# garrelt/C2-Ray3Dm

Hardware: AMD Instinct MI355X
Metric: cells-traced/sec (grid^3 x sources / wallclock) on 256^3 (higher is better)
Workload: dtype f64

## Files before the change

c2-ray3dm_amd/_capi.py:

```python
import ctypes as C
import os

_HERE = os.path.dirname(os.path.abspath(__file__))
LIB_PATH = os.path.join(_HERE, "libc2ray_hip.so")
MAX_ITER_LOG = 128

GRID_NDENS, GRID_XH, GRID_XH_AV, GRID_XH_INTERMED, GRID_PHIH, GRID_PHIHEAT, GRID_TEMPER, GRID_XH0, GRID_XH_AV0, GRID_XH_INTERMED0 = range(10)


class Params(C.Structure):
    _fields_ = [("mesh", C.c_int32 * 3), ("device", C.c_int32), ("subboxsize", C.c_int32),
                ("max_subbox", C.c_int32), ("numtau", C.c_int32), ("max_outer_iter", C.c_int32),
                ("max_chem_iter", C.c_int32), ("deterministic_rates", C.c_int32),
                ("sweep_mode", C.c_int32), ("allfrac", C.c_int32),
                ("epsilon", C.c_double), ("convergence_fraction", C.c_double),
                ("minimum_fractional_change", C.c_double), ("minimum_fraction_of_atoms", C.c_double),
                ("loss_fraction", C.c_double), ("max_coldensh", C.c_double),
                ("tau_photo_limit", C.c_double), ("sigma_HI", C.c_double),
                ("minlogtau", C.c_double), ("dlogtau", C.c_double), ("weight_floor", C.c_double),
                ("sqrt2", C.c_double), ("sqrt3", C.c_double), ("pi", C.c_double),
                ("abu_c", C.c_double), ("bh00", C.c_double), ("albpow", C.c_double),
                ("colh0", C.c_double), ("temph0", C.c_double), ("S_star", C.c_double),
                ("scratch_bytes", C.c_size_t)]

# ... 55 lines not shown
    ("c2r_set_clumping_grid", C.c_int, [_P, _P]),
    ("c2r_default_thermal", C.c_int, [C.POINTER(ThermalParams)]),
    ("c2r_set_thermal", C.c_int, [_P, C.POINTER(ThermalParams), _P, _P, _I32, _P]),
    ("c2r_set_redshift", C.c_int, [_P, _D]),
    ("c2r_set_final_temperature", C.c_int, [_P]),
    ("c2r_set_sources", C.c_int, [_P, _P, _P, _I32]),
    ("c2r_set_exchange_overlap", C.c_int, [_P, _I32]),
    ("c2r_set_xray_tables", C.c_int, [_P, _P, _P, _I32]),
    ("c2r_set_xray_heat_tables", C.c_int, [_P, _P, _P, _I32]),
    ("c2r_set_xray_sources", C.c_int, [_P, _P, _I32]),
    ("c2r_set_rank", C.c_int, [_P, _I32, _I32, ALLREDUCE_FN, _P]),
    ("c2r_set_slab_chemistry", C.c_int, [_P, _P, _P, _P]),
    ("c2r_slab", C.c_int, [_P, _I32, _I32, C.POINTER(C.c_size_t), C.POINTER(C.c_size_t)]),
    ("c2r_set_source_share", C.c_int, [_P, _P, _I32]),
    ("c2r_last_nbox", C.c_int, [_P, _P, _I32]),
    ("c2r_set_balance", C.c_int, [_P, _I32]),
    ("c2r_source_share", C.c_int, [_P, _P, _I32, C.POINTER(_I32)]),
    ("c2r_balanced_shares", C.c_int, [_P, _I32, _I32, _I32, _P, C.POINTER(_I32)]),
    ("c2r_set_source_queue", C.c_int, [_P, _P, _P, _I32]),
    ("c2r_get_device", C.c_int, [_P, C.POINTER(_I32)]),
    ("c2r_bind_device_buffers", C.c_int, [_P, _P, _P, _P, _P, _P]),
    ("c2r_device_ptr", C.c_int, [_P, _I32, C.POINTER(_P)]),
    ("c2r_upload", C.c_int, [_P, _I32, _P]),
    ("c2r_download", C.c_int, [_P, _I32, _P]),
    ("c2r_zero_rates", C.c_int, [_P]),
    ("c2r_pass_sources", C.c_int, [_P, C.POINTER(_D), C.POINTER(_I64), C.POINTER(_I64)]),
    ("c2r_allreduce_rates", C.c_int, [_P]),
    ("c2r_exchange_stats", C.c_int, [_P, C.POINTER(_I64), C.POINTER(_I64), C.POINTER(_I64), C.POINTER(_I64)]),
    ("c2r_evolve0d_host", C.c_int, [_P, _I32, C.c_void_p, C.c_void_p, C.c_void_p, C.c_void_p, C.c_void_p, C.c_void_p, C.c_void_p,
                                    C.c_void_p, C.POINTER(_D)]),
# ... 96 lines not shown
```

c2-ray3dm_amd/csrc/ctx.hpp:

```cpp
#pragma once
#include "../../include/c2ray_hip.h"
#include "../../include/c2ray_constants.h"
#include "kernels_common.hpp"

#include <algorithm>
#include <chrono>
#include <cmath>
#include <cstdio>
#include <cstring>
#include <functional>
#include <map>
#include <string>
#include <vector>

namespace c2r {

struct BoxDesc;

constexpr int kSumBlocks = 1024;
constexpr int kFoldLossMax = 64;
constexpr int kFusedQmax = 10;
constexpr int kMaxSlabRanks = 64;
constexpr int kFewSources = 32;

constexpr int kMaxChains = 4;
struct SweepScratch {
    hipStream_t stream = nullptr; bool own_stream = false;
    int cap = 0;
    double *d_planes = nullptr;
    double *d_gbox = nullptr;
    double *d_gbox_h = nullptr;
    int *d_srcpos_b = nullptr, *d_srcw_b = nullptr; double *d_nflux_b = nullptr, *d_nflux_x = nullptr;
    char *d_batch = nullptr, *h_batch = nullptr; size_t batch_bytes = 0;
    char *d_batch_init = nullptr; std::vector<char> batch_image;
    char *d_hbatch = nullptr;
    int *d_active[2] = {nullptr, nullptr};
    int *d_nactive = nullptr;
    int *h_nactive = nullptr;
    int *d_hnactive = nullptr;
    std::vector<hipEvent_t> ev_box;
    hipEvent_t ev_done = nullptr;
    double *d_loss_partial = nullptr, *d_loss_acc = nullptr, *d_final_loss = nullptr;
    int *d_final_nbox = nullptr;
    int *d_perm = nullptr, *h_perm = nullptr;
};

struct Ctx {
    c2r_params prm{};
    hipStream_t stream = nullptr;
    bool own_stream = false;
    size_t ncell = 0;
    void *grid[10] = {nullptr, nullptr, nullptr, nullptr, nullptr, nullptr, nullptr, nullptr, nullptr, nullptr};
// ... 8 lines not shown
    bool  own[5] = {false, false, false, false, false};
    double *d_thick = nullptr, *d_thin = nullptr;
    v2f64 *d_logtab = nullptr;
    v2f64 *d_odtab = nullptr;
    bool fast = false;
    bool have_tables = false, have_step = false;
    double dr[3] = {0, 0, 0}, vol = 0, lls = 0, temper = 0;
    float clumping = 1.0f;
    std::vector<int32_t> srcpos;
    std::vector<double>  nflux;
    bool xray = false; std::vector<double> nflux_x; double *d_xthick = nullptr, *d_xthin = nullptr;
    bool have_xheat = false; double *d_xhthick = nullptr, *d_xhthin = nullptr;
    int nsrc = 0, rank = 0, nranks = 1;
    bool explicit_share = false; std::vector<int32_t> share;
    std::vector<int32_t> last_nbox;
    int box_hint = 0;
    struct BatchGraph { hipGraph_t graph = nullptr; hipGraphExec_t exec = nullptr; unsigned long long gen = 0; int count = 0, n_active = 0, hint = 0;
                        bool fused = false; bool stats = false; const void *acc = nullptr;
    };
    std::map<int, BatchGraph> graphs;
    struct ChainGraph { hipGraph_t graph = nullptr; hipGraphExec_t exec = nullptr; unsigned long long gen = 0; int count = 0, n_active = 0, shape_count = 0;
                        const void *acc = nullptr; bool perm = false; int H = 0, launches = 0; std::vector<int> bounds, profile, profile_prev; int passes_since_capture = 0; };
    std::map<int, ChainGraph> chain_graphs;
    bool chain_tail = true;
    bool chain_graph = true;
    long long chain_replays = 0, chain_halts = 0, chain_eager = 0;
    unsigned long long gen = 1;
    long long captures = 0;
    bool use_graph = true;
    bool fused_iter = true;
// ... 125 lines not shown
```

c2-ray3dm_amd/csrc/kernels_sweep.hpp:

```cpp
#pragma once
#include "kernels_common.hpp"

namespace c2r {

template <int EXT>
__device__ __forceinline__ void source_cell(const KParams &p, const v2f64 *__restrict__ ltab, const int s, const bool on_surface,
                                            double *loss_acc, double *dbg_cdout)
{
    const int i = pmod(p.srcpos[3 * s + 0] - 1, p.n[0]);
    const int j = pmod(p.srcpos[3 * s + 1] - 1, p.n[1]);
    const int k = pmod(p.srcpos[3 * s + 2] - 1, p.n[2]);
    const size_t id = (size_t)i + (size_t)p.n[0] * ((size_t)j + (size_t)p.n[1] * (size_t)k);
    const double nhi = p.nhi[id];
    const double cd_in = 0.0;
    const double path = 0.5 * step_of(p).dr[0];
    const double vol_ph = step_of(p).dr[0] * step_of(p).dr[1] * step_of(p).dr[2];
    const double cd_out = cd_in + nhi * path;
    for (int f = 0; f < 6; ++f)
        p.planes[((size_t)s * 2 + 0) * 6 * p.PP + (size_t)f * p.PP + (size_t)p.R * p.P + p.R] = cd_out;
    if (dbg_cdout) dbg_cdout[id] = cd_out;
    const double nflux = p.normflux[s];
    double p_out = 0.0, gamma = 0.0;
    if (nflux > 0.0) {
        double heat = 0.0;
// ... 601 lines not shown
    __shared__ v2f64 s_log[kBlock];
    const int face = blockIdx.y;
    const int tile = blockIdx.x;
    const int nact = *sa.n_active;
    if ((int)blockIdx.z >= nact) return;
    const FaceRect fr = sa.face[face];
    if (tile >= fr.ntiles && !sa.has_boundary) return;
    const v2f64 *ltab = wave_log_table(p.odtab, s_log);
    sweep_tile_fast<DET, LLS, STREAM, EXT>(p, sa, fr, ltab, p.thick, sm, face, tile, (int)blockIdx.z, sa);
}

struct XcdArgs {
    const int *perm;
    int n, cap;
    const int *final_nbox;
};
template <bool DET, int LLS, bool STREAM, int EXT, bool FAST>
__global__ C2R_FAST_ATTR void k_sweep_shell_xcd(KParams p, ShellArgs sa, XcdArgs xa)
{
    __shared__ double sm[16];
    __shared__ v2f64 s_log[kBlock];
    const unsigned x = blockIdx.x & 7u;
    unsigned r = blockIdx.x >> 3;
    const unsigned start = (x * (unsigned)xa.n) >> 3, cnt = (((x + 1u) * (unsigned)xa.n) >> 3) - start;
    int face = -1; unsigned item = 0, tile = 0;
#pragma unroll
    for (int f = 0; f < 6; ++f) {
        const unsigned nt = (unsigned)sa.face[f].ntiles, nb = cnt * nt;
        if (face < 0) {
            if (r < nb) { face = f; item = r / nt; tile = r - item * nt; }
            else r -= nb;
        }
    }
    if (face < 0) return;
    const int s = xa.perm[(2 - (face >> 1)) * xa.cap + (int)(start + item)];
    if (xa.final_nbox[s] != 0) return;
    const FaceRect fr = sa.face[face];
    const v2f64 *ltab = wave_log_table(p.odtab, s_log);
    if (FAST) sweep_tile_fast<DET, LLS, STREAM ? 3 : 2, EXT>(p, sa, fr, ltab, p.thick, sm, face, (int)tile, 0, sa, s);
    else sweep_tile<DET, LLS, STREAM ? 3 : 2, EXT>(p, sa, fr, ltab, sm, face, (int)tile, 0, sa, s);
}

template <bool DET, int LLS, bool STREAM, int EXT>
__global__ __launch_bounds__(kBlock) __attribute__((amdgpu_waves_per_eu(1, 4)))
void k_sweep_pair_fast(KParams p, ShellArgs sa, ShellArgs sb)
{
    __shared__ double sm[16];
    __shared__ v2f64 s_log[kBlock];
    const bool second = blockIdx.y >= 6;
    const int face = second ? (int)blockIdx.y - 6 : (int)blockIdx.y;
    const int tile = blockIdx.x;
    const int nact = *sa.n_active;
    if ((int)blockIdx.z >= nact) return;
    const v2f64 *ltab = (C2R_PAIR_LDS_TABLE) ? wave_log_table(p.odtab, s_log) : p.odtab;
    if (second) {
// ... 214 lines not shown
                                                     int bps, double *loss_acc)
{
    __shared__ double sm[4];
    const int sl = blockIdx.x;
    if (sl >= *n_active) return;
    double v = 0.0;
    for (int i = threadIdx.x; i < bps; i += 256) v += loss_partial[(size_t)sl * bps + i];
    const double tot = block_sum_256(v, sm);
    if (threadIdx.x == 0) loss_acc[active[sl]] += tot;
}

__global__ __launch_bounds__(1024) void k_box_decide(const int *active_in, const int *n_in_dev, int *active_out,
                                                     int *n_out, int *n_out_host, const double *normflux, double S_star,
                                                     double loss_fraction, int can_grow, int nbox,
                                                     double *loss_acc, double *final_loss, int *final_nbox,
                                                     const double *loss_partial, int bps, int next_bound, int *halt_host)
{
    __shared__ int scan[1024];
    __shared__ int base;
    const int n_in = *n_in_dev;
    if (threadIdx.x == 0) base = 0;
    __syncthreads();
    for (int start = 0; start < n_in; start += 1024) {
        const int i = start + (int)threadIdx.x;
        int keep = 0, s = -1;
        if (i < n_in) {
            s = active_in[i];
            const double flux = normflux[s] * S_star;
            double loss = loss_acc[s];
            if (bps > 0) {
                const double *pp = loss_partial + (size_t)i * bps;
// ... 5 lines not shown
                loss_acc[s] = loss;
            }
            keep = (loss > loss_fraction * flux) && can_grow;
            if (keep) loss_acc[s] = 0.0;
            else { final_loss[s] = loss; final_nbox[s] = nbox; }
        }
        scan[threadIdx.x] = keep;
        __syncthreads();
        for (int off = 1; off < 1024; off <<= 1) {
            int v = 0;
            if ((int)threadIdx.x >= off) v = scan[threadIdx.x - off];
            __syncthreads();
            scan[threadIdx.x] += v;
            __syncthreads();
        }
        if (keep) active_out[base + scan[threadIdx.x] - 1] = s;
        __syncthreads();
        if (threadIdx.x == 1023) base += scan[1023];
        __syncthreads();
    }
    if (threadIdx.x == 0) {
        const bool over = base > next_bound;
        *n_out = over ? 0 : base; *n_out_host = base;
        if (over) *halt_host = nbox;
    }
}

struct SmallTotals {
    int on, nsrc;
    double *photon_loss; long long *sum_nbox;
    double *host_loss; long long *host_nbox;
    int *host_final_nbox; double *host_final_loss;
};
__global__ __launch_bounds__(64) void k_box_decide_small(const int *active_in, const int *n_in_dev, int *active_out,
                                                         int *n_out, int *n_out_host, const double *normflux, double S_star,
                                                         double loss_fraction, int can_grow, int nbox,
                                                         double *loss_acc, double *final_loss, int *final_nbox,
                                                         const double *loss_partial, int bps, SmallTotals tot,
                                                         int next_bound, int *halt_host)
{
#if defined(__AMDGCN_WAVEFRONT_SIZE) && __AMDGCN_WAVEFRONT_SIZE != 64
#error "k_box_decide_small is one 64-lane wave (ballot, cross-lane reads of final_loss): build for a wave64 target (gfx950)"
#endif
    const int n_in = *n_in_dev;
    const int i = threadIdx.x;
    int keep = 0, s = -1;
    if (i < n_in) {
        s = active_in[i];
        const double flux = normflux[s] * S_star;
        double loss = loss_acc[s];
        if (bps > 0) {
            const double *pp = loss_partial + (size_t)i * bps;
            double a0 = 0.0, a1 = 0.0, a2 = 0.0, a3 = 0.0;
            int j = 0;
            for (; j + 3 < bps; j += 4) { a0 += pp[j]; a1 += pp[j + 1]; a2 += pp[j + 2]; a3 += pp[j + 3]; }
            for (; j < bps; ++j) a0 += pp[j];
            loss = loss + ((a0 + a1) + (a2 + a3));
            loss_acc[s] = loss;
        }
        keep = (loss > loss_fraction * flux) && can_grow;
        if (keep) loss_acc[s] = 0.0;
        else { final_loss[s] = loss; final_nbox[s] = nbox; }
    }
    const unsigned long long mask = __ballot(keep);
    if (keep) active_out[__popcll(mask & ((1ULL << i) - 1ULL))] = s;
    const int n_keep = __popcll(mask);
    if (i == 0) {
        const bool over = n_keep > next_bound;
        *n_out = over ? 0 : n_keep; *n_out_host = n_keep;
        if (over) *halt_host = nbox;
    }
    if (tot.on && n_keep == 0) {
        __threadfence_block();
        __syncthreads();
        for (int t = i; t < tot.nsrc; t += 64) { tot.host_final_nbox[t] = final_nbox[t]; tot.host_final_loss[t] = final_loss[t]; }
        if (i == 0) {
            double L = 0.0; long long NB = 0;
            for (int t = 0; t < tot.nsrc; ++t) { L = L + (0.0 + final_loss[t]); NB += final_nbox[t]; }
            *tot.photon_loss = L; *tot.sum_nbox = NB;
            *tot.host_loss = L; *tot.host_nbox = NB;
// ... 38 lines not shown
```

c2-ray3dm_amd/csrc/sweep.hip:

```cpp
#include "ctx.hpp"
#include "kernels_sweep.hpp"
#include <climits>

namespace c2r {

namespace {
void free_chain(SweepScratch &sc)
{
    hipFree(sc.d_planes); hipFree(sc.d_gbox); hipFree(sc.d_gbox_h); hipFree(sc.d_batch); hipFree(sc.d_batch_init); hipFree(sc.d_loss_partial);
    hipFree(sc.d_perm);
    if (sc.h_perm) hipHostFree(sc.h_perm);
    if (sc.h_batch) hipHostFree(sc.h_batch);
    if (sc.h_nactive) hipHostFree(sc.h_nactive);
    for (auto &e : sc.ev_box) hipEventDestroy(e);
    if (sc.ev_done) hipEventDestroy(sc.ev_done);
    const hipStream_t st = sc.stream; const bool own = sc.own_stream;
    sc = SweepScratch();
    sc.stream = st; sc.own_stream = own;
}
}

void free_sweep_scratch(Ctx *ctx)
{
    for (int c = 0; c < kMaxChains; ++c) free_chain(ctx->sc[c]);
// ... 11 lines not shown
{
    if (ctx->chains_env > 0) return std::min(ctx->chains_env, std::max(1, want));
    if (ctx->prm.deterministic_rates || want < 64 || want > 768) return 1;
    if (ctx->stream_hint && ctx->xcd_order != 0 &&
        (double)want >= ctx->xcd_min_per_plane * (double)std::min(ctx->prm.mesh[0], std::min(ctx->prm.mesh[1], ctx->prm.mesh[2]))) return 1;
    return (want >= 192 && want <= 384) ? 3 : 2;
}

int alloc_chain(Ctx *ctx, SweepScratch &sc, int cap)
{
    if (!sc.stream) { HIP_TRY(hipStreamCreateWithFlags(&sc.stream, hipStreamNonBlocking)); sc.own_stream = true; }
    HIP_TRY(hipMalloc(&sc.d_planes, (size_t)cap * 2 * 6 * ctx->PP * sizeof(double)));
    if (ctx->prm.deterministic_rates) HIP_TRY(hipMalloc(&sc.d_gbox, (size_t)cap * 2 * ctx->ncell * sizeof(double)));
    if (ctx->prm.deterministic_rates && ctx->thermal) HIP_TRY(hipMalloc(&sc.d_gbox_h, (size_t)cap * 2 * ctx->ncell * sizeof(double)));
    HIP_TRY(hipMalloc(&sc.d_loss_partial, (size_t)cap * 6 * ctx->tiles_cap * sizeof(double)));
    sc.batch_bytes = (size_t)cap * 4 * sizeof(double) + ((size_t)cap * 9 + 2) * sizeof(int);
    HIP_TRY(hipMalloc(&sc.d_batch, sc.batch_bytes));
    HIP_TRY(hipMalloc(&sc.d_batch_init, sc.batch_bytes));
    sc.batch_image.clear();
    HIP_TRY(hipHostMalloc((void **)&sc.h_batch, sc.batch_bytes, hipHostMallocMapped));
    HIP_TRY(hipHostGetDevicePointer((void **)&sc.d_hbatch, sc.h_batch, 0));
    {
        double *d = reinterpret_cast<double *>(sc.d_batch);
        sc.d_nflux_b = d; sc.d_final_loss = d + cap; sc.d_loss_acc = d + 2 * (size_t)cap; sc.d_nflux_x = d + 3 * (size_t)cap;
        int *i = reinterpret_cast<int *>(d + 4 * (size_t)cap);
        sc.d_srcpos_b = i; sc.d_srcw_b = i + 3 * (size_t)cap; sc.d_active[0] = i + 6 * (size_t)cap;
        sc.d_active[1] = i + 7 * (size_t)cap; sc.d_final_nbox = i + 8 * (size_t)cap; sc.d_nactive = i + 9 * (size_t)cap;
    }
    HIP_TRY(hipMalloc(&sc.d_perm, (size_t)3 * cap * sizeof(int)));
    HIP_TRY(hipHostMalloc((void **)&sc.h_perm, (size_t)3 * cap * sizeof(int)));
    HIP_TRY(hipHostMalloc((void **)&sc.h_nactive, (size_t)(ctx->nbox_max + 2) * sizeof(int), hipHostMallocMapped));
    HIP_TRY(hipHostGetDevicePointer((void **)&sc.d_hnactive, sc.h_nactive, 0));
    sc.ev_box.resize(ctx->nbox_max + 2);
    for (auto &e : sc.ev_box) HIP_TRY(hipEventCreateWithFlags(&e, hipEventDisableTiming));
    HIP_TRY(hipEventCreateWithFlags(&sc.ev_done, hipEventDisableTiming));
    sc.cap = cap;
    return C2R_OK;
}
}

int ensure_sweep_scratch(Ctx *ctx, int want)
{
// ... 187 lines not shown
        if ((spins & 63u) == 63u && std::chrono::steady_clock::now() - t0 > std::chrono::microseconds(500)) {
            (void)hipGetLastError();
            HIP_TRY(hipEventSynchronize(ev));
            return C2R_OK;
        }
        cpu_relax();
    }
    (void)hipGetLastError();
    return C2R_OK;
}

struct BatchSweep {
    Ctx *ctx; SweepScratch &sc; const c2r_params &p;
    const int first, count; const bool first_of_pass; double *const dbg; FusedIter *const fz;
    const size_t cap; hipStream_t st; KParams k;
    double *h_nf, *h_fl, *h_nfx; int *h_pos, *h_posw, *h_act, *h_na, *h_fnb;
    int n_active = 0;
    int cur = 0, last_bps = 0;
    int totals_at_box = 0;

    const int shape_count;
    bool chained = false;
    int launches = 0;
    int bound = 0, known = 0;
    int next = 1, last = 0;
    bool perm_ready = false;

    BatchSweep(Ctx *c, SweepScratch &sc_, int first_, int count_, bool first_of_pass_, double *dbg_, FusedIter *fz_)
        : ctx(c), sc(sc_), p(c->prm), first(first_), count(count_), first_of_pass(first_of_pass_), dbg(dbg_), fz(fz_),
          cap((size_t)sc_.cap), st(sc_.stream), k(make_kparams(c, sc_)), shape_count(c->queue_next ? c->nsrc : n_local_sources(c))
    {
        h_nf = reinterpret_cast<double *>(sc.h_batch); h_fl = h_nf + cap; h_nfx = h_nf + 3 * cap;
        h_pos = reinterpret_cast<int *>(h_nf + 4 * cap); h_posw = h_pos + 3 * cap; h_act = h_pos + 6 * cap; h_na = h_pos + 9 * cap;
        h_fnb = h_pos + 8 * cap;
    }

    void stage()
    {
        memset(sc.h_batch, 0, sc.batch_bytes);
        const bool can_trace = ctx->hr[2] > 0 && ctx->hl[2] > 0;
        n_active = 0;
        for (int i = 0; i < count; ++i) {
            const int g = ctx->explicit_share ? ctx->share[first + i]
                                              : ctx->rank + (first + i) * ctx->nranks;
            for (int d = 0; d < 3; ++d) {
                h_pos[3 * i + d] = ctx->srcpos[3 * (size_t)g + d];
                const int m = (h_pos[3 * i + d] - 1) % p.mesh[d];
                h_posw[3 * i + d] = m < 0 ? m + p.mesh[d] : m;
            }
            h_nf[i] = ctx->nflux[g];
            h_nfx[i] = (ctx->xray && g < (int)ctx->nflux_x.size()) ? ctx->nflux_x[g] : 0.0;
            const double flux = h_nf[i] * p.S_star;
            if (flux > p.loss_fraction * flux && can_trace) h_act[n_active++] = i;
            else h_fl[i] = flux;
        }
        h_na[0] = n_active; h_na[1] = 0;
    }

    void stage_perm()
    {
        perm_ready = false;
        if (dbg || !sc.d_perm || ctx->xcd_order == 0 || n_active < ctx->xcd_min_sources) return;
        const int nmin = std::min(p.mesh[0], std::min(p.mesh[1], p.mesh[2]));
        if (ctx->xcd_order < 0 && (double)n_active < ctx->xcd_min_per_plane * (double)nmin * (sc.d_gbox ? 0.5 : 1.0)) return;
        for (int d = 0; d < 3; ++d) {
            int *perm = sc.h_perm + (size_t)d * cap;
            for (int t = 0; t < n_active; ++t) perm[t] = h_act[t];
            std::stable_sort(perm, perm + n_active, [&](int a, int b) { return h_posw[3 * a + d] < h_posw[3 * b + d]; });
// ... 143 lines not shown
                        case 4: C2R_LAUNCH_PAIR(false, 2); break;
                        case 5: C2R_LAUNCH_PAIR(true, 2); break;
                        case 6: C2R_LAUNCH_PAIR(false, 3); break;
                        default: C2R_LAUNCH_PAIR(true, 3); break;
                    }
#undef C2R_LAUNCH_PAIR
#undef C2R_LAUNCH_PAIR_H
                    pbuf = 1 - pbuf;
                    ++q;
                    continue;
                }
            }
            pbuf = 1 - pbuf;
            ++in_box;
            if (prof == 1) prof_begin(ctx, ctx->ev_sweep, ctx->ev_sweep_used);
            if (perm_ready && !sa.has_boundary && q >= ctx->xcd_qmin && (double)bound >= ctx->xcd_min_alive * (double)n_active) {
                XcdArgs xa{};
                xa.perm = sc.d_perm; xa.n = n_active; xa.cap = (int)cap; xa.final_nbox = sc.d_final_nbox;
                int tiles6 = 0;
                for (int f = 0; f < 6; ++f) tiles6 += sa.face[f].ntiles;
                const dim3 grid(8u * (unsigned)((n_active + 7) / 8) * (unsigned)tiles6), blk(kBlock);
#define C2R_LAUNCH_XCD_D(D, L, H, F) do { if (ctx->stream_hint) hipLaunchKernelGGL((k_sweep_shell_xcd<D, L, true, H, F>), grid, blk, 0, st, k, sa, xa); \
                                          else hipLaunchKernelGGL((k_sweep_shell_xcd<D, L, false, H, F>), grid, blk, 0, st, k, sa, xa); } while (0)
#define C2R_LAUNCH_XCD_F(L, H, F) do { if (det) C2R_LAUNCH_XCD_D(true, L, H, F); else C2R_LAUNCH_XCD_D(false, L, H, F); } while (0)
#define C2R_LAUNCH_XCD_H(L, H) do { if (ctx->fast) C2R_LAUNCH_XCD_F(L, H, true); else C2R_LAUNCH_XCD_F(L, H, false); } while (0)
#define C2R_LAUNCH_XCD(L) do { if (ctx->thermal && ctx->xray) C2R_LAUNCH_XCD_H(L, 3); else if (ctx->thermal) C2R_LAUNCH_XCD_H(L, 1); else if (ctx->xray) C2R_LAUNCH_XCD_H(L, 2); else C2R_LAUNCH_XCD_H(L, 0); } while (0)
                switch (ctx->lls_type) {
                    case 1: C2R_LAUNCH_XCD(1); break;
                    case 2: C2R_LAUNCH_XCD(2); break;
                    default: C2R_LAUNCH_XCD(3); break;
                }
#undef C2R_LAUNCH_XCD
#undef C2R_LAUNCH_XCD_H
// ... 35 lines not shown
    {
        const int nbox = bx.nbox;
        int *const halt = sc.d_hnactive;
        const int can_grow = (p.subboxsize * nbox < ctx->hr[2]) && (p.subboxsize * nbox < ctx->hl[2]);
        if (n_active <= 64) {
            SmallTotals tot{};
            if (nbox == totals_at_box) {
                tot.on = 1; tot.nsrc = count; tot.photon_loss = ctx->d_photon_loss; tot.sum_nbox = ctx->d_sum_nbox;
                tot.host_loss = &ctx->d_hsc->photon_loss; tot.host_nbox = &ctx->d_hsc->sum_nbox;
                tot.host_final_loss = reinterpret_cast<double *>(sc.d_hbatch) + cap;
                tot.host_final_nbox = reinterpret_cast<int *>(reinterpret_cast<double *>(sc.d_hbatch) + 4 * cap) + 8 * cap;
            }
            hipLaunchKernelGGL(k_box_decide_small, dim3(1), dim3(64), 0, st, sc.d_active[cur], sc.d_nactive + cur,
                               sc.d_active[1 - cur], sc.d_nactive + (1 - cur), sc.d_hnactive + nbox, sc.d_nflux_b,
                               p.S_star, p.loss_fraction, can_grow, nbox, sc.d_loss_acc, sc.d_final_loss, sc.d_final_nbox,
                               (const double *)sc.d_loss_partial, last_bps, tot, bx.next_bound, halt);
        } else
        hipLaunchKernelGGL(k_box_decide, dim3(1), dim3(1024), 0, st, sc.d_active[cur], sc.d_nactive + cur,
                           sc.d_active[1 - cur], sc.d_nactive + (1 - cur), sc.d_hnactive + nbox, sc.d_nflux_b,
                           p.S_star, p.loss_fraction, can_grow, nbox, sc.d_loss_acc, sc.d_final_loss, sc.d_final_nbox,
                           (const double *)sc.d_loss_partial, last_bps, bx.next_bound, halt);
    }

    int enqueue_box(const int nbox, const int bound, const int next_bound = INT_MAX)
    {
        Box bx{};
        bx.nbox = nbox; bx.bound = bound; bx.next_bound = next_bound;
        for (int d = 0; d < 3; ++d) {
            bx.boxR[d] = std::min(p.subboxsize * nbox, ctx->hr[d]);
            bx.boxL[d] = std::min(p.subboxsize * nbox, ctx->hl[d]);
        }
        bx.pair_ok = ctx->pair_shells && n_active <= kFewSources && !dbg && ctx->prof != 1;
        bx.pbuf = plane_set_before(ctx, nbox, n_active, bx.pair_ok);
        bx.fused_box = box_is_fused(ctx, nbox, bx.pair_ok);
        bx.q0 = p.subboxsize * (nbox - 1) + 1; bx.q1 = std::min(p.subboxsize * nbox, ctx->Qmax);
        bx.det = sc.d_gbox != nullptr;
// ... 164 lines not shown
        cg.perm = perm_ready;
        cg.passes_since_capture = 0;
        return true;
    }
    if (cg.graph) { hipGraphDestroy(cg.graph); cg.graph = nullptr; }
    cg.exec = nullptr;
    (void)hipGetLastError();
    ctx->use_graph = false;
    return false;
}

int sweep_batch(Ctx *ctx, int first, int count, bool first_of_pass, double *dbg, std::vector<int> *nbox_out,
                std::vector<double> *loss_out, FusedIter *fz = nullptr)
{
    BatchSweep bs(ctx, ctx->sc[0], first, count, first_of_pass, dbg, fz);
    return bs.run(nbox_out, loss_out);
}

#ifndef C2R_CHAIN_AHEAD
#define C2R_CHAIN_AHEAD 2
#endif
constexpr int kChainAhead = C2R_CHAIN_AHEAD;

static void bounds_from_profile(const std::vector<int> &prof, int n_active, std::vector<int> &bounds, int &H)
{
    H = 0;
    while (H + 1 < (int)prof.size() && prof[H] > 0) ++H;
    bounds.assign((size_t)H + 1, 0);
    for (int nb = 1; nb <= H; ++nb) {
        const int c = prof[nb - 1];
// ... 14 lines not shown
        have += cg.bounds[nb]; need += cg.profile[nb - 1];
    }
    return have <= need + need / 2 + 4LL * H;
}

static_assert(kFusedQmaxK == kFusedQmax, "the fused kernel's LDS planes are sized for kFusedQmax");
static_assert(kGateChains >= kMaxChains, "k_chain_gate holds every chain's pointers");
int run_chains(Ctx *ctx, int first, int count, bool first_of_pass, std::vector<int> *nbox_out, FusedIter *tail)
{
    const int nch = std::min(ctx->nchains, count);
    const int per = (count + nch - 1) / nch;
    std::vector<BatchSweep> ch;
    ch.reserve(nch);
    for (int c = 0, f = first; c < nch && f < first + count; ++c, f += per)
        ch.emplace_back(ctx, ctx->sc[c], f, std::min(per, first + count - f), first_of_pass && c == 0, nullptr, nullptr);
    HIP_TRY(hipEventRecord(ctx->ev_prepared, ctx->stream));
    if (ctx->prof) prof_begin(ctx, ctx->ev_sweep, ctx->ev_sweep_used);
    std::vector<Ctx::ChainGraph *> graph_of(ch.size(), nullptr);
    for (size_t c = 0; c < ch.size(); ++c) {
        BatchSweep &b = ch[c];
        b.chained = true;
        b.stage();
        if (ctx->xcd_order > 0) b.stage_perm();
        if (b.st != ctx->stream) HIP_TRY(hipStreamWaitEvent(b.st, ctx->ev_prepared, 0));
        b.bound = b.n_active; b.known = 0; b.cur = 0; b.next = 1;
        Ctx::ChainGraph &cg = ctx->chain_graphs[b.first];
        ++cg.passes_since_capture;
        bool replay = false;
        if (ctx->use_graph && ctx->chain_graph && b.n_active > 0 && !cg.profile.empty()) {
            replay = chain_graph_fits(ctx, cg, b, (const void *)b.k.phih);
// ... 207 lines not shown
    ctx->xchg_bytes_total += ctx->xchg_bytes_last;
    return C2R_OK;
}
}

int pass_sources_impl(Ctx *ctx, FusedIter *fz, double *photon_loss, int64_t *sum_nbox, int64_t *visited, bool no_wait, FusedIter *chain_tail)
{
    int rc;
    if ((rc = sync_step(ctx))) return rc;
    const bool queued = ctx->queue_next != nullptr && fz == nullptr;
    if (queued) { ctx->share.clear(); ctx->explicit_share = true; ctx->auto_share = true; }
    else balance_before_pass(ctx);
    int nloc = queued ? 0 : n_local_sources(ctx);
    long long vis = 0;
    ++ctx->pass_id; ctx->sparse_valid = ctx->rates_clean || fz != nullptr; ctx->rates_clean = false;
    ctx->last_nbox.clear();
    ctx->h_sc->photon_loss = 0.0; ctx->h_sc->sum_nbox = 0;
    const bool overlap = !queued && exchange_overlap_applies(ctx, fz);
    if (queued) {
        bool prepared = false;
        std::vector<int> nb;
        for (;;) {
            int32_t qf = 0, qc = 0;
            if (ctx->queue_next(ctx->queue_user, (int64_t)ctx->pass_id, ctx->queue_chunk, &qf, &qc) != 0) FAIL(C2R_ECALLBACK, "source queue callback failed");
            if (qc <= 0) break;
            if (qf < 0 || qc > ctx->queue_chunk || qf + qc > ctx->nsrc) FAIL(C2R_ECALLBACK, "source queue handed out sources beyond the list");
            const int first = (int)ctx->share.size();
            for (int i = 0; i < qc; ++i) ctx->share.push_back(qf + i);
            if ((rc = ensure_sweep_scratch(ctx, ctx->queue_chunk))) return rc;
            if (!prepared) { if ((rc = sweep_prepare(ctx))) return rc; prepared = true; }
            for (int f = first, count = 0; f < first + qc; f += count) {
// ... 60 lines not shown
}

using namespace c2r;

extern "C" {

int c2r_pass_sources(c2r_ctx *c, double *photon_loss, int64_t *sum_nbox, int64_t *visited)
{
    if (!c) return C2R_EINVAL;
    Ctx *ctx = C(c);
    int rc = check_ready(ctx);
    if (rc) return rc;
    return pass_sources_impl(ctx, nullptr, photon_loss, sum_nbox, visited);
}

int c2r_do_source(c2r_ctx *c, int32_t ns, double *cd_host, double *loss, int32_t *nbox, int64_t *visited)
{
    if (!c) return C2R_EINVAL;
    Ctx *ctx = C(c);
    int rc = check_ready(ctx);
    if (rc) return rc;
    if (ns < 1 || ns > ctx->nsrc) FAIL(C2R_EINVAL, "source number out of range");
    rc = ensure_sweep_scratch(ctx, 1);
    if (rc) return rc;
    if ((rc = sync_step(ctx))) return rc;
    ctx->sparse_valid = false; ctx->rates_clean = false;
    double *dbg = nullptr;
    if (cd_host) {
        if (!ctx->d_dbg) HIP_TRY(hipMalloc(&ctx->d_dbg, ctx->ncell * sizeof(double)));
        HIP_TRY(hipMemsetAsync(ctx->d_dbg, 0, ctx->ncell * sizeof(double), ctx->stream));
// ... 1 lines not shown
    }
    const int sr = ctx->rank, sn = ctx->nranks;
    const bool se = ctx->explicit_share;
    ctx->rank = 0; ctx->nranks = 1; ctx->explicit_share = false;
    std::vector<int> nb; std::vector<double> fl;
    rc = sweep_prepare(ctx);
    if (!rc) rc = sweep_batch(ctx, ns - 1, 1, true, dbg, &nb, &fl);
    if (!rc) rc = sweep_finish(ctx);
    ctx->rank = sr; ctx->nranks = sn; ctx->explicit_share = se;
    if (rc) return rc;
    prof_collect(ctx);
    if (cd_host) {
        HIP_TRY(hipMemcpyAsync(cd_host, ctx->d_dbg, ctx->ncell * sizeof(double), hipMemcpyDeviceToHost, ctx->stream));
        HIP_TRY(hipStreamSynchronize(ctx->stream));
    }
    if (loss) *loss = fl[0];
    if (nbox) *nbox = nb[0];
    if (visited) *visited = visited_for_nbox(ctx, nb[0]);
    return C2R_OK;
}

int c2r_evolve0d_host(c2r_ctx *c, int32_t ns, const int32_t rtpos[3], const int32_t last_l[3], const int32_t last_r[3],
                      const float *ndens, const double *xh_av, double *coldensh_out, double *phih_grid, double *phiheat_grid,
                      double *photon_loss_src)
{
    if (!c || !rtpos || !last_l || !last_r || !ndens || !xh_av || !coldensh_out || !phih_grid) return C2R_EINVAL;
    Ctx *ctx = C(c);
    int rc = check_ready(ctx);
    if (rc) return rc;
    if (ns < 1 || ns > ctx->nsrc) FAIL(C2R_EINVAL, "source number out of range");
// ... 79 lines not shown
```

c2-ray3dm_amd/evolve.py:

```python
import ctypes as C
import os
import time as _time
import numpy as np

from . import _capi
from ._capi import C2RayHipError



def static_source_share(nsrc, rank, npr):
    return list(range(rank, nsrc, npr))


def box_cost(nbox, mesh, subbox=5):
    v = np.ones_like(np.asarray(nbox), dtype=np.int64)
    for n in mesh:
        hr, hl = n // 2 - 1 + n % 2, n // 2
        v = v * (np.minimum(subbox * np.asarray(nbox), hr) + np.minimum(subbox * np.asarray(nbox), hl) + 1)
    return np.where(np.asarray(nbox) > 0, v, 0)


def balanced_source_shares(cost, npr):
    cost = np.asarray(cost, dtype=np.int64)
    order = sorted(range(len(cost)), key=lambda i: (-int(cost[i]), i))
# ... 155 lines not shown
    def set_balance(self, on=True):
        self._check(self.lib.c2r_set_balance(self.ctx, 1 if on else 0), "c2r_set_balance")

    def local_sources(self):
        n = C.c_int32()
        idx = np.zeros(max(1, self.nsrc), dtype=np.int32)
        self._check(self.lib.c2r_source_share(self.ctx, idx.ctypes.data, idx.size, C.byref(n)), "c2r_source_share")
        return idx[:n.value].astype(np.int64)

    def last_nbox(self):
        n = len(self.local_sources())
        out = np.zeros(n, dtype=np.int32)
        self._check(self.lib.c2r_last_nbox(self.ctx, out.ctypes.data, n), "c2r_last_nbox")
        return out

    def set_rank(self, rank, npr, allreduce=None):
        self.rank, self.npr = rank, npr
        if npr > 1:
            torch = self.torch
            known = {self.phih_grid.data_ptr(): self.phih_grid}

            def _cb(user, ptr, count, stream):
                try:
                    t = known.get(ptr)
                    if t is None:
                        t = torch.as_tensor(_DevView(ptr, count), device=self.device)
                    if stream:
                        with torch.cuda.stream(torch.cuda.ExternalStream(stream, device=self.device)):
                            allreduce(t)
                    else:
# ... 406 lines not shown
```

include/c2ray_hip.h:

```cpp
#ifndef C2RAY_HIP_H
#define C2RAY_HIP_H

#include <stddef.h>
#include <stdint.h>

#ifdef __cplusplus
extern "C" {
#endif
#if defined(__GNUC__) || defined(__clang__)
#pragma GCC visibility push(default)
#endif

#define C2R_OK            0
#define C2R_EINVAL      (-1)
#define C2R_ESTATE      (-2)
#define C2R_ENOMEM      (-3)
#define C2R_ECALLBACK   (-4)

#define C2R_MAX_ITER_LOG 128

#define C2R_DEVICE_AUTO  (-1)
#define C2R_SWEEP_EXACT   0
#define C2R_SWEEP_FAST    1

// ... 90 lines not shown
int  c2r_set_redshift(c2r_ctx *ctx, double zred);
int  c2r_set_final_temperature(c2r_ctx *ctx);

int  c2r_set_sources(c2r_ctx *ctx, const int32_t *srcpos, const double *normflux, int32_t nsrc);
int  c2r_set_rank(c2r_ctx *ctx, int32_t rank, int32_t nranks, c2r_allreduce_fn fn, void *user);

typedef int (*c2r_reduce_scatter_fn)(void *user, void *dev_buf, const size_t *elem_offset, const size_t *elem_count,
                                     int32_t nranks, void *hip_stream);
typedef int (*c2r_allgather_fn)(void *user, void *dev_buf, const size_t *byte_offset, const size_t *byte_count,
                                int32_t nranks, void *hip_stream);
int  c2r_set_slab_chemistry(c2r_ctx *ctx, c2r_reduce_scatter_fn rs, c2r_allgather_fn ag, void *user);
int  c2r_slab(const c2r_ctx *ctx, int32_t rank, int32_t nranks, size_t *cell_offset, size_t *cell_count);

int  c2r_set_source_share(c2r_ctx *ctx, const int32_t *idx, int32_t n);
int  c2r_last_nbox(c2r_ctx *ctx, int32_t *nbox, int32_t n);
int  c2r_set_balance(c2r_ctx *ctx, int32_t on);
int  c2r_source_share(c2r_ctx *ctx, int32_t *idx, int32_t cap, int32_t *n);
int  c2r_balanced_shares(const int64_t *cost, int32_t nsrc, int32_t nranks, int32_t rank, int32_t *idx, int32_t *n);
typedef int (*c2r_next_sources_fn)(void *user, int64_t pass, int32_t want, int32_t *first, int32_t *count);
int  c2r_set_source_queue(c2r_ctx *ctx, c2r_next_sources_fn next, void *user, int32_t chunk);
int  c2r_get_device(const c2r_ctx *ctx, int32_t *device);

int  c2r_bind_device_buffers(c2r_ctx *ctx, void *ndens, void *xh, void *xh_av,
                             void *xh_intermed, void *phih_grid);
int  c2r_device_ptr(c2r_ctx *ctx, int32_t which, void **ptr);
int  c2r_upload(c2r_ctx *ctx, int32_t which, const void *host);
int  c2r_download(c2r_ctx *ctx, int32_t which, void *host);

int  c2r_zero_rates(c2r_ctx *ctx);
int  c2r_pass_sources(c2r_ctx *ctx, double *photon_loss, int64_t *sum_nbox, int64_t *visited);
// ... 70 lines not shown
```

Before: 123.4 billion.

## Enable XCD-permuted shell sweep for boundary boxes via per-source slot map

Adds a slot_of array, filled by the box-decide kernels and host init, that maps each source to its compacted active slot. The XCD-permuted shell sweep can then write per-slot photon-loss partials, so the restriction that skipped the XCD path when the box touches a boundary is removed. The kernel also zeroes unused loss-partial tiles and returns early when no sources are active. A new c2r_last_loss API exposes per-source final losses. The gain from running the permuted path in more boxes is paid for with extra slot writes and reads and the tile-zeroing loop.

```diff
diff --git a/c2-ray3dm_amd/_capi.py b/c2-ray3dm_amd/_capi.py
--- a/c2-ray3dm_amd/_capi.py
+++ b/c2-ray3dm_amd/_capi.py
@@ -93,6 +93,7 @@
     ("c2r_slab", C.c_int, [_P, _I32, _I32, C.POINTER(C.c_size_t), C.POINTER(C.c_size_t)]),
     ("c2r_set_source_share", C.c_int, [_P, _P, _I32]),
     ("c2r_last_nbox", C.c_int, [_P, _P, _I32]),
+    ("c2r_last_loss", C.c_int, [_P, _P, _I32]),
     ("c2r_set_balance", C.c_int, [_P, _I32]),
     ("c2r_source_share", C.c_int, [_P, _P, _I32, C.POINTER(_I32)]),
     ("c2r_balanced_shares", C.c_int, [_P, _I32, _I32, _I32, _P, C.POINTER(_I32)]),
diff --git a/c2-ray3dm_amd/csrc/ctx.hpp b/c2-ray3dm_amd/csrc/ctx.hpp
--- a/c2-ray3dm_amd/csrc/ctx.hpp
+++ b/c2-ray3dm_amd/csrc/ctx.hpp
@@ -36,6 +36,7 @@
     char *d_hbatch = nullptr;
     int *d_active[2] = {nullptr, nullptr};
     int *d_nactive = nullptr;
+    int *d_slot_of = nullptr;
     int *h_nactive = nullptr;
     int *d_hnactive = nullptr;
     std::vector<hipEvent_t> ev_box;
@@ -74,6 +75,7 @@
     int nsrc = 0, rank = 0, nranks = 1;
     bool explicit_share = false; std::vector<int32_t> share;
     std::vector<int32_t> last_nbox;
+    std::vector<std::pair<int, int>> loss_parts; int loss_rounds = 0;
     int box_hint = 0;
     struct BatchGraph { hipGraph_t graph = nullptr; hipGraphExec_t exec = nullptr; unsigned long long gen = 0; int count = 0, n_active = 0, hint = 0;
                         bool fused = false; bool stats = false; const void *acc = nullptr;
diff --git a/c2-ray3dm_amd/csrc/kernels_sweep.hpp b/c2-ray3dm_amd/csrc/kernels_sweep.hpp
--- a/c2-ray3dm_amd/csrc/kernels_sweep.hpp
+++ b/c2-ray3dm_amd/csrc/kernels_sweep.hpp
@@ -639,6 +639,7 @@
     const int *perm;
     int n, cap;
     const int *final_nbox;
+    const int *slot_of;
 };
 template <bool DET, int LLS, bool STREAM, int EXT, bool FAST>
 __global__ C2R_FAST_ATTR void k_sweep_shell_xcd(KParams p, ShellArgs sa, XcdArgs xa)
@@ -658,12 +659,26 @@
         }
     }
     if (face < 0) return;
+    if (*sa.n_active == 0) return;
     const int s = xa.perm[(2 - (face >> 1)) * xa.cap + (int)(start + item)];
     if (xa.final_nbox[s] != 0) return;
+    const int sl = sa.has_boundary ? xa.slot_of[s] : 0;
     const FaceRect fr = sa.face[face];
     const v2f64 *ltab = wave_log_table(p.odtab, s_log);
-    if (FAST) sweep_tile_fast<DET, LLS, STREAM ? 3 : 2, EXT>(p, sa, fr, ltab, p.thick, sm, face, (int)tile, 0, sa, s);
-    else sweep_tile<DET, LLS, STREAM ? 3 : 2, EXT>(p, sa, fr, ltab, sm, face, (int)tile, 0, sa, s);
+    if (FAST) sweep_tile_fast<DET, LLS, STREAM ? 3 : 2, EXT>(p, sa, fr, ltab, p.thick, sm, face, (int)tile, sl, sa, s);
+    else sweep_tile<DET, LLS, STREAM ? 3 : 2, EXT>(p, sa, fr, ltab, sm, face, (int)tile, sl, sa, s);
+    if (sa.has_boundary && tile == 0) {
+        int f0 = 0;
+#pragma unroll
+        for (int f = 5; f >= 0; --f) f0 = sa.face[f].ntiles > 0 ? f : f0;
+        double *const lp = sa.loss_partial + (size_t)sl * 6 * sa.tiles_max;
+#pragma unroll
+        for (int f = 0; f < 6; ++f) {
+            const int nt = sa.face[f].ntiles;
+            if (f == face || (nt == 0 && face == f0))
+                for (int t = nt + (int)threadIdx.x; t < sa.tiles_max; t += kBlock) lp[f * sa.tiles_max + t] = 0.0;
+        }
+    }
 }
 
 template <bool DET, int LLS, bool STREAM, int EXT>
@@ -908,7 +923,8 @@
                                                      int *n_out, int *n_out_host, const double *normflux, double S_star,
                                                      double loss_fraction, int can_grow, int nbox,
                                                      double *loss_acc, double *final_loss, int *final_nbox,
-                                                     const double *loss_partial, int bps, int next_bound, int *halt_host)
+                                                     const double *loss_partial, int bps, int next_bound, int *halt_host,
+                                                     int *slot_of )
 {
     __shared__ int scan[1024];
     __shared__ int base;
@@ -944,7 +960,7 @@
             scan[threadIdx.x] += v;
             __syncthreads();
         }
-        if (keep) active_out[base + scan[threadIdx.x] - 1] = s;
+        if (keep) { active_out[base + scan[threadIdx.x] - 1] = s; slot_of[s] = base + scan[threadIdx.x] - 1; }
         __syncthreads();
         if (threadIdx.x == 1023) base += scan[1023];
         __syncthreads();
@@ -967,7 +983,7 @@
                                                          double loss_fraction, int can_grow, int nbox,
                                                          double *loss_acc, double *final_loss, int *final_nbox,
                                                          const double *loss_partial, int bps, SmallTotals tot,
-                                                         int next_bound, int *halt_host)
+                                                         int next_bound, int *halt_host, int *slot_of )
 {
 #if defined(__AMDGCN_WAVEFRONT_SIZE) && __AMDGCN_WAVEFRONT_SIZE != 64
 #error "k_box_decide_small is one 64-lane wave (ballot, cross-lane reads of final_loss): build for a wave64 target (gfx950)"
@@ -993,7 +1009,7 @@
         else { final_loss[s] = loss; final_nbox[s] = nbox; }
     }
     const unsigned long long mask = __ballot(keep);
-    if (keep) active_out[__popcll(mask & ((1ULL << i) - 1ULL))] = s;
+    if (keep) { active_out[__popcll(mask & ((1ULL << i) - 1ULL))] = s; slot_of[s] = __popcll(mask & ((1ULL << i) - 1ULL)); }
     const int n_keep = __popcll(mask);
     if (i == 0) {
         const bool over = n_keep > next_bound;
diff --git a/c2-ray3dm_amd/csrc/sweep.hip b/c2-ray3dm_amd/csrc/sweep.hip
--- a/c2-ray3dm_amd/csrc/sweep.hip
+++ b/c2-ray3dm_amd/csrc/sweep.hip
@@ -49,7 +49,7 @@
     if (ctx->prm.deterministic_rates) HIP_TRY(hipMalloc(&sc.d_gbox, (size_t)cap * 2 * ctx->ncell * sizeof(double)));
     if (ctx->prm.deterministic_rates && ctx->thermal) HIP_TRY(hipMalloc(&sc.d_gbox_h, (size_t)cap * 2 * ctx->ncell * sizeof(double)));
     HIP_TRY(hipMalloc(&sc.d_loss_partial, (size_t)cap * 6 * ctx->tiles_cap * sizeof(double)));
-    sc.batch_bytes = (size_t)cap * 4 * sizeof(double) + ((size_t)cap * 9 + 2) * sizeof(int);
+    sc.batch_bytes = (size_t)cap * 4 * sizeof(double) + ((size_t)cap * 10 + 2) * sizeof(int);
     HIP_TRY(hipMalloc(&sc.d_batch, sc.batch_bytes));
     HIP_TRY(hipMalloc(&sc.d_batch_init, sc.batch_bytes));
     sc.batch_image.clear();
@@ -61,6 +61,7 @@
         int *i = reinterpret_cast<int *>(d + 4 * (size_t)cap);
         sc.d_srcpos_b = i; sc.d_srcw_b = i + 3 * (size_t)cap; sc.d_active[0] = i + 6 * (size_t)cap;
         sc.d_active[1] = i + 7 * (size_t)cap; sc.d_final_nbox = i + 8 * (size_t)cap; sc.d_nactive = i + 9 * (size_t)cap;
+        sc.d_slot_of = i + 9 * (size_t)cap + 2;
     }
     HIP_TRY(hipMalloc(&sc.d_perm, (size_t)3 * cap * sizeof(int)));
     HIP_TRY(hipHostMalloc((void **)&sc.h_perm, (size_t)3 * cap * sizeof(int)));
@@ -278,7 +279,7 @@
     Ctx *ctx; SweepScratch &sc; const c2r_params &p;
     const int first, count; const bool first_of_pass; double *const dbg; FusedIter *const fz;
     const size_t cap; hipStream_t st; KParams k;
-    double *h_nf, *h_fl, *h_nfx; int *h_pos, *h_posw, *h_act, *h_na, *h_fnb;
+    double *h_nf, *h_fl, *h_nfx; int *h_pos, *h_posw, *h_act, *h_na, *h_fnb, *h_slot;
     int n_active = 0;
     int cur = 0, last_bps = 0;
     int totals_at_box = 0;
@@ -296,6 +297,7 @@
     {
         h_nf = reinterpret_cast<double *>(sc.h_batch); h_fl = h_nf + cap; h_nfx = h_nf + 3 * cap;
         h_pos = reinterpret_cast<int *>(h_nf + 4 * cap); h_posw = h_pos + 3 * cap; h_act = h_pos + 6 * cap; h_na = h_pos + 9 * cap;
+        h_slot = h_na + 2;
         h_fnb = h_pos + 8 * cap;
     }
 
@@ -315,7 +317,7 @@
             h_nf[i] = ctx->nflux[g];
             h_nfx[i] = (ctx->xray && g < (int)ctx->nflux_x.size()) ? ctx->nflux_x[g] : 0.0;
             const double flux = h_nf[i] * p.S_star;
-            if (flux > p.loss_fraction * flux && can_trace) h_act[n_active++] = i;
+            if (flux > p.loss_fraction * flux && can_trace) { h_slot[i] = n_active; h_act[n_active++] = i; }
             else h_fl[i] = flux;
         }
         h_na[0] = n_active; h_na[1] = 0;
@@ -489,9 +491,9 @@
             pbuf = 1 - pbuf;
             ++in_box;
             if (prof == 1) prof_begin(ctx, ctx->ev_sweep, ctx->ev_sweep_used);
-            if (perm_ready && !sa.has_boundary && q >= ctx->xcd_qmin && (double)bound >= ctx->xcd_min_alive * (double)n_active) {
+            if (perm_ready && q >= ctx->xcd_qmin && (double)bound >= ctx->xcd_min_alive * (double)n_active) {
                 XcdArgs xa{};
-                xa.perm = sc.d_perm; xa.n = n_active; xa.cap = (int)cap; xa.final_nbox = sc.d_final_nbox;
+                xa.perm = sc.d_perm; xa.n = n_active; xa.cap = (int)cap; xa.final_nbox = sc.d_final_nbox; xa.slot_of = sc.d_slot_of;
                 int tiles6 = 0;
                 for (int f = 0; f < 6; ++f) tiles6 += sa.face[f].ntiles;
                 const dim3 grid(8u * (unsigned)((n_active + 7) / 8) * (unsigned)tiles6), blk(kBlock);
@@ -557,12 +559,12 @@
             hipLaunchKernelGGL(k_box_decide_small, dim3(1), dim3(64), 0, st, sc.d_active[cur], sc.d_nactive + cur,
                                sc.d_active[1 - cur], sc.d_nactive + (1 - cur), sc.d_hnactive + nbox, sc.d_nflux_b,
                                p.S_star, p.loss_fraction, can_grow, nbox, sc.d_loss_acc, sc.d_final_loss, sc.d_final_nbox,
-                               (const double *)sc.d_loss_partial, last_bps, tot, bx.next_bound, halt);
+                               (const double *)sc.d_loss_partial, last_bps, tot, bx.next_bound, halt, sc.d_slot_of);
         } else
         hipLaunchKernelGGL(k_box_decide, dim3(1), dim3(1024), 0, st, sc.d_active[cur], sc.d_nactive + cur,
                            sc.d_active[1 - cur], sc.d_nactive + (1 - cur), sc.d_hnactive + nbox, sc.d_nflux_b,
                            p.S_star, p.loss_fraction, can_grow, nbox, sc.d_loss_acc, sc.d_final_loss, sc.d_final_nbox,
-                           (const double *)sc.d_loss_partial, last_bps, bx.next_bound, halt);
+                           (const double *)sc.d_loss_partial, last_bps, bx.next_bound, halt, sc.d_slot_of);
     }
 
     int enqueue_box(const int nbox, const int bound, const int next_bound = INT_MAX)
@@ -757,6 +759,7 @@
                 std::vector<double> *loss_out, FusedIter *fz = nullptr)
 {
     BatchSweep bs(ctx, ctx->sc[0], first, count, first_of_pass, dbg, fz);
+    ++ctx->loss_rounds; ctx->loss_parts.assign(1, std::make_pair(0, count));
     return bs.run(nbox_out, loss_out);
 }
 
@@ -801,6 +804,8 @@
     ch.reserve(nch);
     for (int c = 0, f = first; c < nch && f < first + count; ++c, f += per)
         ch.emplace_back(ctx, ctx->sc[c], f, std::min(per, first + count - f), first_of_pass && c == 0, nullptr, nullptr);
+    ++ctx->loss_rounds; ctx->loss_parts.clear();
+    for (size_t c = 0; c < ch.size(); ++c) ctx->loss_parts.emplace_back((int)c, ch[c].count);
     HIP_TRY(hipEventRecord(ctx->ev_prepared, ctx->stream));
     if (ctx->prof) prof_begin(ctx, ctx->ev_sweep, ctx->ev_sweep_used);
     std::vector<Ctx::ChainGraph *> graph_of(ch.size(), nullptr);
@@ -1038,7 +1043,7 @@
     int nloc = queued ? 0 : n_local_sources(ctx);
     long long vis = 0;
     ++ctx->pass_id; ctx->sparse_valid = ctx->rates_clean || fz != nullptr; ctx->rates_clean = false;
-    ctx->last_nbox.clear();
+    ctx->last_nbox.clear(); ctx->loss_parts.clear(); ctx->loss_rounds = 0;
     ctx->h_sc->photon_loss = 0.0; ctx->h_sc->sum_nbox = 0;
     const bool overlap = !queued && exchange_overlap_applies(ctx, fz);
     if (queued) {
@@ -1129,6 +1134,22 @@
     return pass_sources_impl(ctx, nullptr, photon_loss, sum_nbox, visited);
 }
 
+int c2r_last_loss(c2r_ctx *c, double *loss, int32_t n)
+{
+    if (!c || (n > 0 && !loss)) return C2R_EINVAL;
+    Ctx *ctx = C(c);
+    if (ctx->loss_rounds != 1) FAIL(C2R_ESTATE, "per-source losses are kept for a pass that ran as one round of launches");
+    int have = 0;
+    for (const auto &pt : ctx->loss_parts) have += pt.second;
+    if (n != have) FAIL(C2R_EINVAL, "length must equal the number of sources this rank swept");
+    int at = 0;
+    for (const auto &pt : ctx->loss_parts) {
+        HIP_TRY(hipMemcpy(loss + at, ctx->sc[pt.first].d_final_loss, (size_t)pt.second * sizeof(double), hipMemcpyDeviceToHost));
+        at += pt.second;
+    }
+    return C2R_OK;
+}
+
 int c2r_do_source(c2r_ctx *c, int32_t ns, double *cd_host, double *loss, int32_t *nbox, int64_t *visited)
 {
     if (!c) return C2R_EINVAL;
@@ -1160,6 +1181,7 @@
         HIP_TRY(hipMemcpyAsync(cd_host, ctx->d_dbg, ctx->ncell * sizeof(double), hipMemcpyDeviceToHost, ctx->stream));
         HIP_TRY(hipStreamSynchronize(ctx->stream));
     }
+    ctx->loss_parts.clear(); ctx->loss_rounds = 0;
     if (loss) *loss = fl[0];
     if (nbox) *nbox = nb[0];
     if (visited) *visited = visited_for_nbox(ctx, nb[0]);
diff --git a/c2-ray3dm_amd/evolve.py b/c2-ray3dm_amd/evolve.py
--- a/c2-ray3dm_amd/evolve.py
+++ b/c2-ray3dm_amd/evolve.py
@@ -193,6 +193,12 @@
         self._check(self.lib.c2r_last_nbox(self.ctx, out.ctypes.data, n), "c2r_last_nbox")
         return out
 
+    def last_loss(self):
+        n = len(self.local_sources())
+        out = np.zeros(n, dtype=np.float64)
+        self._check(self.lib.c2r_last_loss(self.ctx, out.ctypes.data, n), "c2r_last_loss")
+        return out
+
     def set_rank(self, rank, npr, allreduce=None):
         self.rank, self.npr = rank, npr
         if npr > 1:
diff --git a/include/c2ray_hip.h b/include/c2ray_hip.h
--- a/include/c2ray_hip.h
+++ b/include/c2ray_hip.h
@@ -128,6 +128,7 @@
 
 int  c2r_set_source_share(c2r_ctx *ctx, const int32_t *idx, int32_t n);
 int  c2r_last_nbox(c2r_ctx *ctx, int32_t *nbox, int32_t n);
+int  c2r_last_loss(c2r_ctx *ctx, double *loss, int32_t n);
 int  c2r_set_balance(c2r_ctx *ctx, int32_t on);
 int  c2r_source_share(c2r_ctx *ctx, int32_t *idx, int32_t cap, int32_t *n);
 int  c2r_balanced_shares(const int64_t *cost, int32_t nsrc, int32_t nranks, int32_t rank, int32_t *idx, int32_t *n);
```

Result: slower. 121.7 billion (-1.4%).
